# amazon-science/glass-text-spotting

Hardware: AMD Instinct MI355X
Metric: images/sec/GPU end-to-end spotting, 1000x1000, ~32 RoIs; 1/2/4/8 GPU scaling (higher is better)
Workload: dtype f32

## Files before the change

glass-text-spotting_amd/csrc/conv.hip:

```cpp
#include "splitk_common.h"
#include "common.h"
#include <cstdlib>

typedef float f32x16 __attribute__((ext_vector_type(16)));

struct ConvParams {
  const float* x;
  const float* w;
  const float* bias;
  const float* res;
  float* y;
  int N, H, W, Cin, Cout, KH, KW, sh, sw, ph, pw, Ho, Wo;
  int ldx, ldy, ycoff, ycs, relu, res_mode, ldr;
  int M, Ktot, nk, tiles_m, tiles_n, vec_epi;
  unsigned x_bytes, w_bytes;
  unsigned y_bytes, r_bytes;
  unsigned magic_cin, magic_kw;
  int ksplit;
  long split_y;
  int half_mode;
  int xh, yh, rh;
};

__device__ __forceinline__ float4 sel4(bool ok, float4 v) {
  return make_float4(ok ? v.x : 0.f, ok ? v.y : 0.f, ok ? v.z : 0.f, ok ? v.w : 0.f);
}


typedef unsigned u32x4 __attribute__((ext_vector_type(4)));
typedef unsigned u32x2 __attribute__((ext_vector_type(2)));

typedef _Float16 h8 __attribute__((ext_vector_type(8)));
typedef _Float16 h4 __attribute__((ext_vector_type(4)));

template <int WAVES_M, int WAVES_N, int TM, int TN, int NSTAGE, int MINW, int BK, int MODE, bool HALF>
__global__ __launch_bounds__(256, MINW) void conv_igemm_f32(ConvParams pin) {
  ConvParams p = pin;
  int kt0 = 0, kt1 = pin.nk;
  if (pin.ksplit > 1) {
    const int per = pin.nk / pin.ksplit;
    kt0 = (int)blockIdx.y * per;
    kt1 = kt0 + per;
    p.y += (long)blockIdx.y * pin.split_y;
  }
  constexpr bool FAST = MODE == 1, BUF = MODE != 0;
  constexpr int LDS_LD = HALF ? BK + 8 : BK + 4;
  constexpr int KCH = BK / 4;
  constexpr int RPP = 256 / KCH;
  constexpr int BM = WAVES_M * TM * 32;
  constexpr int BN = WAVES_N * TN * 32;
  constexpr int A_LOADS = BM / RPP;
  constexpr int B_LOADS = BN / RPP;
  constexpr int STAGE = (BM + BN) * LDS_LD;
  constexpr int ESZ = HALF ? 2 : 4;
  constexpr int CW = (NSTAGE * STAGE * ESZ >= BM * 68 * 4 && BN >= 64) ? 64 : 32;
  constexpr int SMEM_BYTES = NSTAGE * STAGE * ESZ > BM * (CW + 4) * 4 ? NSTAGE * STAGE * ESZ : BM * (CW + 4) * 4;
  __shared__ __attribute__((aligned(16))) unsigned char smem_raw[SMEM_BYTES];
  float* smem = reinterpret_cast<float*>(smem_raw);
  _Float16* hmem = reinterpret_cast<_Float16*>(smem_raw);

  const int nblk = gridDim.x, bid = blockIdx.x;
  const int xcd = bid & 7, q = nblk >> 3, r = nblk & 7;
  const int logical = (xcd < r ? xcd * (q + 1) : r * (q + 1) + (xcd - r) * q) + (bid >> 3);
  const int tile_m = logical / p.tiles_n;
  const int tile_n = logical - tile_m * p.tiles_n;
  const int m0 = tile_m * BM, n0 = tile_n * BN;

  const int tid = threadIdx.x, lane = tid & 63, wave = tid >> 6;
  const int wm = wave / WAVES_N, wn = wave % WAVES_N;
  const int cc = tid % KCH;
  const int r0 = tid / KCH;

  long a_base[A_LOADS];
  int a_hi0[A_LOADS], a_wi0[A_LOADS];
// ... 117 lines not shown
      float4 v = *reinterpret_cast<const float4*>(src);
      areg[i] = sel4(ok, v);
    }
#pragma unroll
    for (int i = 0; i < B_LOADS; ++i) {
      const bool ok = kvalid && b_ok[i];
      const float* src = ok ? (p.w + b_off[i] + (long)kt * BK) : p.w;
      float4 v = *reinterpret_cast<const float4*>(src);
      breg[i] = sel4(ok, v);
    }
  };
  auto load_tile = [&](int kt) {
    if constexpr (MODE == 1) load_tile_fast(kt); else if constexpr (MODE == 2) load_tile_buf(kt); else load_tile_generic(kt);
  };
  auto store_tile = [&](int stage) {
    if constexpr (HALF) {
      _Float16* As = hmem + stage * STAGE;
      _Float16* Bs = As + BM * LDS_LD;
      auto to_h4 = [](float4 v) { return h4{(_Float16)v.x, (_Float16)v.y, (_Float16)v.z, (_Float16)v.w}; };
#pragma unroll
      for (int i = 0; i < A_LOADS; ++i)
        *reinterpret_cast<h4*>(&As[(r0 + RPP * i) * LDS_LD + cc * 4]) = to_h4(areg[i]);
#pragma unroll
      for (int i = 0; i < B_LOADS; ++i)
        *reinterpret_cast<h4*>(&Bs[(r0 + RPP * i) * LDS_LD + cc * 4]) = to_h4(breg[i]);
    } else {
      float* As = smem + stage * STAGE;
      float* Bs = As + BM * LDS_LD;
#pragma unroll
      for (int i = 0; i < A_LOADS; ++i)
        *reinterpret_cast<float4*>(&As[(r0 + RPP * i) * LDS_LD + cc * 4]) = areg[i];
// ... 5 lines not shown

  f32x16 acc[TM][TN];
#pragma unroll
  for (int i = 0; i < TM; ++i)
#pragma unroll
    for (int j = 0; j < TN; ++j)
#pragma unroll
      for (int e = 0; e < 16; ++e) acc[i][j][e] = 0.f;

  const int frag_row = lane & 31;
  const int frag_k = (lane >> 5) * 4;
  const float* a_frag0 = smem + (wm * TM * 32 + frag_row) * LDS_LD + frag_k;
  const float* b_frag0 = smem + BM * LDS_LD + (wn * TN * 32 + frag_row) * LDS_LD + frag_k;
  const _Float16* a_frag0h = hmem + (wm * TM * 32 + frag_row) * LDS_LD + (lane >> 5) * 8;
  const _Float16* b_frag0h = hmem + BM * LDS_LD + (wn * TN * 32 + frag_row) * LDS_LD + (lane >> 5) * 8;

  load_tile(kt0);
  store_tile(0);
  __syncthreads();
  for (int kt = kt0; kt < kt1; ++kt) {
    const bool more = kt + 1 < kt1;
    if (BUF || more) load_tile(kt + 1);
    const int cur = NSTAGE == 2 ? ((kt - kt0) & 1) : 0;
    if constexpr (HALF) {
      const _Float16* a_frag = a_frag0h + cur * STAGE;
      const _Float16* b_frag = b_frag0h + cur * STAGE;
#pragma unroll
      for (int g = 0; g < BK / 16; ++g) {
        h8 af[TM], bf[TN];
#pragma unroll
        for (int i = 0; i < TM; ++i) af[i] = *reinterpret_cast<const h8*>(a_frag + i * 32 * LDS_LD + g * 16);
#pragma unroll
        for (int j = 0; j < TN; ++j) bf[j] = *reinterpret_cast<const h8*>(b_frag + j * 32 * LDS_LD + g * 16);
#pragma unroll
        for (int i = 0; i < TM; ++i)
#pragma unroll
          for (int j = 0; j < TN; ++j) acc[i][j] = __builtin_amdgcn_mfma_f32_32x32x16_f16(af[i], bf[j], acc[i][j], 0, 0, 0);
      }
    } else {
// ... 9 lines not shown
#pragma unroll
      for (int s = 0; s < 4; ++s) {
#pragma unroll
        for (int i = 0; i < TM; ++i) {
          const float a = s == 0 ? af[i].x : s == 1 ? af[i].y : s == 2 ? af[i].z : af[i].w;
#pragma unroll
          for (int j = 0; j < TN; ++j) {
            const float b = s == 0 ? bf[j].x : s == 1 ? bf[j].y : s == 2 ? bf[j].z : bf[j].w;
            acc[i][j] = __builtin_amdgcn_mfma_f32_32x32x2f32(a, b, acc[i][j], 0, 0, 0);
          }
        }
      }
    }
    }
    if constexpr (BUF) {
      constexpr int NL = A_LOADS + B_LOADS, NM = HALF ? (BK / 16) * TM * TN : (BK / 8) * 4 * TM * TN, PER = NM / NL > 0 ? NM / NL : 1;
#pragma unroll
      for (int i = 0; i < NL; ++i) {
        __builtin_amdgcn_sched_group_barrier(0x020, 1, 0);
        __builtin_amdgcn_sched_group_barrier(0x008, PER, 0);
      }
    }
    if (NSTAGE == 2) {
      if (more) store_tile((kt + 1 - kt0) & 1);
      __syncthreads();
    } else {
      __syncthreads();
      if (more) {
        store_tile(0);
        __syncthreads();
      }
// ... 124 lines not shown
  }
}

template <int WAVES_M, int WAVES_N, int TM, int TN, int NSTAGE, int MINW, int BK, bool HALF>
static int launch_conv_cfg(ConvParams& p, hipStream_t stream) {
  constexpr int BM = WAVES_M * TM * 32, BN = WAVES_N * TN * 32;
  p.tiles_m = cdiv(p.M, BM);
  p.tiles_n = cdiv(p.Cout, BN);
  const long nblk = (long)p.tiles_m * p.tiles_n;
  if (nblk <= 0 || nblk > 0x7fffffffL) {
    glass_set_error("glass_conv2d_nhwc: bad grid %ld", nblk);
    return GLASS_EINVAL;
  }
  p.nk = cdiv(p.Ktot, BK);
  const dim3 grid((unsigned)nblk, (unsigned)(p.ksplit > 1 ? p.ksplit : 1));
  if (p.x_bytes != 0 && p.Cin % BK == 0)
    hipLaunchKernelGGL((conv_igemm_f32<WAVES_M, WAVES_N, TM, TN, NSTAGE, MINW, BK, 1, HALF>), grid, dim3(256), 0, stream, p);
  else if (p.x_bytes != 0)
    hipLaunchKernelGGL((conv_igemm_f32<WAVES_M, WAVES_N, TM, TN, NSTAGE, MINW, BK, 2, HALF>), grid, dim3(256), 0, stream, p);
  else if constexpr (!HALF)
    hipLaunchKernelGGL((conv_igemm_f32<WAVES_M, WAVES_N, TM, TN, NSTAGE, MINW, BK, 0, false>), grid, dim3(256), 0, stream, p);
  else {
    glass_set_error("glass_conv2d_nhwc_f16: tensors of 2 GiB and more are not supported in the fp16 mode");
    return GLASS_EINVAL;
  }
  GLASS_CHECK_LAUNCH("glass_conv2d_nhwc");
  return GLASS_OK;
}

template <int WAVES_M, int WAVES_N, int TM, int TN, int NSTAGE, int MINW, int BK>
static int launch_conv_impl(ConvParams& p, hipStream_t stream) {
  return p.half_mode ? launch_conv_cfg<WAVES_M, WAVES_N, TM, TN, NSTAGE, MINW, BK, true>(p, stream)
                     : launch_conv_cfg<WAVES_M, WAVES_N, TM, TN, NSTAGE, MINW, BK, false>(p, stream);
}

static int conv_dispatch(const glass_conv_desc* d, const float* x, const float* w, const float* bias, const float* residual,
                         float* y, glass_stream_t stream, int half_mode, int h16_flags = 0);

extern "C" int glass_conv2d_nhwc(const glass_conv_desc* d, const float* x, const float* w, const float* bias,
                                 const float* residual, float* y, glass_stream_t stream) {
  return conv_dispatch(d, x, w, bias, residual, y, stream, 0);
}

extern "C" int glass_conv2d_nhwc_f16(const glass_conv_desc* d, const float* x, const float* w, const float* bias,
                                     const float* residual, float* y, glass_stream_t stream) {
  return conv_dispatch(d, x, w, bias, residual, y, stream, 1);
}

extern "C" int glass_conv2d_nhwc_h16(const glass_conv_desc* d, const void* x, const float* w, const float* bias,
                                     const void* residual, void* y, int flags, glass_stream_t stream) {
  GLASS_CHECK_ARG((flags & ~7) == 0, "glass_conv2d_nhwc_h16: unknown flags 0x%x", flags);
  return conv_dispatch(d, static_cast<const float*>(x), w, bias, static_cast<const float*>(residual), static_cast<float*>(y),
                       stream, 1, flags);
}

static int conv_dispatch(const glass_conv_desc* d, const float* x, const float* w, const float* bias, const float* residual,
                         float* y, glass_stream_t stream, int half_mode, int h16_flags) {
  GLASS_CHECK_ARG(d && x && w && y, "glass_conv2d_nhwc: null pointer");
  GLASS_CHECK_ARG(d->Cin > 0 && d->Cin % 4 == 0, "glass_conv2d_nhwc: Cin=%d must be a positive multiple of 4", d->Cin);
  GLASS_CHECK_ARG(d->ldx % 4 == 0 && d->ldx >= d->Cin, "glass_conv2d_nhwc: ldx=%d", d->ldx);
  GLASS_CHECK_ARG(d->N >= 0 && d->H > 0 && d->W > 0 && d->Cout > 0 && d->KH > 0 && d->KW > 0, "glass_conv2d_nhwc: bad dims");
  GLASS_CHECK_ARG(d->stride_h > 0 && d->stride_w > 0, "glass_conv2d_nhwc: bad stride");
  GLASS_CHECK_ARG(d->Ho == (d->H + 2 * d->pad_h - d->KH) / d->stride_h + 1 &&
                      d->Wo == (d->W + 2 * d->pad_w - d->KW) / d->stride_w + 1,
                  "glass_conv2d_nhwc: Ho/Wo (%d,%d) inconsistent with input/kernel/stride/pad", d->Ho, d->Wo);
  GLASS_CHECK_ARG(d->y_cstride >= 1 && d->ldy >= 1 && d->y_coff >= 0, "glass_conv2d_nhwc: bad output strides");
  GLASS_CHECK_ARG((long)d->y_coff + (long)(d->Cout - 1) * d->y_cstride < (long)d->ldy,
                  "glass_conv2d_nhwc: output channel window (y_coff=%d, Cout=%d, y_cstride=%d) exceeds ldy=%d", d->y_coff,
                  d->Cout, d->y_cstride, d->ldy);
  GLASS_CHECK_ARG(d->res_mode == 0 || d->ldr >= d->Cout, "glass_conv2d_nhwc: residual ldr=%d < Cout=%d", d->ldr, d->Cout);
  GLASS_CHECK_ARG(d->res_mode == 0 || residual != nullptr, "glass_conv2d_nhwc: res_mode set but residual is null");
  GLASS_CHECK_ARG(d->res_mode != 2 || (d->Ho % 2 == 0 && d->Wo % 2 == 0), "glass_conv2d_nhwc: upsampled residual needs even Ho/Wo");
  GLASS_CHECK_ARG(((uintptr_t)x & 15) == 0 && ((uintptr_t)w & 15) == 0, "glass_conv2d_nhwc: x/w must be 16-byte aligned");
  if (d->N == 0) return GLASS_OK;
  ConvParams p;
  p.half_mode = half_mode;
  p.xh = h16_flags & 1; p.yh = (h16_flags >> 1) & 1; p.rh = (h16_flags >> 2) & 1;
  const long xes = p.xh ? 2 : 4, yes = p.yh ? 2 : 4, res_ = p.rh ? 2 : 4;
  p.x = x; p.w = w; p.bias = bias; p.res = residual; p.y = y;
  p.N = d->N; p.H = d->H; p.W = d->W; p.Cin = d->Cin; p.Cout = d->Cout; p.KH = d->KH; p.KW = d->KW;
  p.sh = d->stride_h; p.sw = d->stride_w; p.ph = d->pad_h; p.pw = d->pad_w; p.Ho = d->Ho; p.Wo = d->Wo;
  p.ldx = d->ldx; p.ldy = d->ldy; p.ycoff = d->y_coff; p.ycs = d->y_cstride; p.relu = d->relu;
  p.res_mode = d->res_mode; p.ldr = d->ldr;
  const long M = (long)d->N * d->Ho * d->Wo;
  GLASS_CHECK_ARG(M < 0x7fffffffL, "glass_conv2d_nhwc: too many output pixels");
  p.M = (int)M;
  p.Ktot = d->KH * d->KW * d->Cin;
  p.ksplit = 1; p.split_y = 0;
  {
    const long xb = (long)d->N * d->H * d->W * d->ldx * 4, wb = (long)d->Cout * p.Ktot * 4;
    const bool small = xb < 0x7fffff00L && wb < 0x7fffff00L;
// ... 55 lines not shown
                                        glass_stream_t stream) {
  GLASS_CHECK_ARG(d && x && w && y && workspace, "glass_conv2d_nhwc_splitk: null pointer");
  GLASS_CHECK_ARG(glass_conv2d_splitk_supported(d, splits),
                  "glass_conv2d_nhwc_splitk: needs Cin %% 32 == 0, (KH KW Cin / 32) %% splits == 0, 2 <= splits <= 32, res_mode 0/1 and "
                  "operands < 2 GiB (got Cin=%d k=%dx%d splits=%d res_mode=%d)", d->Cin, d->KH, d->KW, splits, d->res_mode);
  GLASS_CHECK_ARG(d->Ho == (d->H + 2 * d->pad_h - d->KH) / d->stride_h + 1 && d->Wo == (d->W + 2 * d->pad_w - d->KW) / d->stride_w + 1,
                  "glass_conv2d_nhwc_splitk: Ho/Wo (%d,%d) inconsistent with input/kernel/stride/pad", d->Ho, d->Wo);
  GLASS_CHECK_ARG(d->y_cstride >= 1 && d->y_coff >= 0 && (long)d->y_coff + (long)(d->Cout - 1) * d->y_cstride < (long)d->ldy,
                  "glass_conv2d_nhwc_splitk: output channel window exceeds ldy=%d", d->ldy);
  GLASS_CHECK_ARG(d->res_mode == 0 || (residual != nullptr && d->ldr >= d->Cout), "glass_conv2d_nhwc_splitk: bad residual");
  GLASS_CHECK_ARG(workspace_bytes >= glass_conv2d_splitk_workspace_bytes(d, splits), "glass_conv2d_nhwc_splitk: workspace too small");
  GLASS_CHECK_ARG((((uintptr_t)x | (uintptr_t)w | (uintptr_t)workspace) & 15) == 0, "glass_conv2d_nhwc_splitk: x / w / workspace must be 16-byte aligned");
  GLASS_CHECK_ARG(d->relu >= 0 && d->relu <= 2, "glass_conv2d_nhwc_splitk: relu must be 0, 1 or 2");
  const long M = (long)d->N * d->Ho * d->Wo;
  ConvParams p;
  p.half_mode = 0; p.xh = p.yh = p.rh = 0;
  p.x = x; p.w = w; p.bias = nullptr; p.res = nullptr; p.y = static_cast<float*>(workspace);
  p.N = d->N; p.H = d->H; p.W = d->W; p.Cin = d->Cin; p.Cout = d->Cout; p.KH = d->KH; p.KW = d->KW;
  p.sh = d->stride_h; p.sw = d->stride_w; p.ph = d->pad_h; p.pw = d->pad_w; p.Ho = d->Ho; p.Wo = d->Wo;
  p.ldx = d->ldx; p.ldy = d->Cout; p.ycoff = 0; p.ycs = 1; p.relu = 0; p.res_mode = 0; p.ldr = 0;
  p.M = (int)M; p.Ktot = d->KH * d->KW * d->Cin; p.ksplit = splits; p.split_y = M * d->Cout;
  p.x_bytes = (unsigned)((long)d->N * d->H * d->W * d->ldx * 4);
  p.w_bytes = (unsigned)((long)d->Cout * p.Ktot * 4);
  p.magic_cin = (unsigned)(0x100000000ULL / (unsigned long long)d->Cin);
  p.magic_kw = (unsigned)(0x100000000ULL / (unsigned long long)d->KW);
  p.vec_epi = d->Cout % 4 == 0 ? 1 : 0;
  p.y_bytes = (unsigned)(M * d->Cout * 4);
  p.r_bytes = 0;
  hipStream_t s = (hipStream_t)stream;
  const int rc = d->Cout <= 32 ? launch_conv_impl<4, 1, 1, 1, 1, 4, 32>(p, s)
                               : launch_conv_impl<2, 2, 1, 1, 1, 8, 32>(p, s);
// ... 7 lines not shown
```

glass-text-spotting_amd/csrc/pointwise_split.hip:

```cpp
#include "wino_common.h"

typedef float f32x4 __attribute__((ext_vector_type(4)));
typedef __bf16 bf16x8 __attribute__((ext_vector_type(8)));
typedef unsigned u32x2 __attribute__((ext_vector_type(2)));

namespace {

constexpr int SN = 128;
constexpr int SK = 32;

struct PwsParams {
  const float* x; const void* u; const float* bias; const float* res; float* y;
  int M, H, W, Ho, Wo, Cin, Cout, stride, nk;
  int ldx, ldy, ycoff, ldr, relu, res_mode;
  int tiles_m, tiles_n;
  unsigned x_bytes, u_bytes, y_bytes, r_bytes;
  unsigned magic_hw, magic_w;
  unsigned long long* dbg;
  const float* x2; int nk1, ldx2; unsigned x2_bytes;
};

#ifdef GLASS_PWS_STAMPS
unsigned long long* g_pws_dbg = nullptr;
#define PWS_STAMP(k) { __builtin_amdgcn_sched_barrier(0); const unsigned long long tn = __builtin_amdgcn_s_memtime(); st[k] += tn - tlast; tlast = tn; __builtin_amdgcn_sched_barrier(0); }
#else
#define PWS_STAMP(k) {}
#endif

typedef float f32x2 __attribute__((ext_vector_type(2)));
typedef __bf16 bf16x2 __attribute__((ext_vector_type(2)));
__device__ __forceinline__ void split3_pair(float v0, float v1, unsigned& hp, unsigned& mp, unsigned& lp) {
  hp = __builtin_bit_cast(unsigned, __builtin_convertvector((f32x2{v0, v1}), bf16x2));
  const float r0 = v0 - __builtin_bit_cast(float, hp << 16), r1 = v1 - __builtin_bit_cast(float, hp & 0xffff0000u);
  mp = __builtin_bit_cast(unsigned, __builtin_convertvector((f32x2{r0, r1}), bf16x2));
  const float l0 = r0 - __builtin_bit_cast(float, mp << 16), l1 = r1 - __builtin_bit_cast(float, mp & 0xffff0000u);
  lp = __builtin_bit_cast(unsigned, __builtin_convertvector((f32x2{l0, l1}), bf16x2));
}

template <int PB, int NPROD, bool DUAL = false>
__global__ __launch_bounds__(256, 2) void conv1x1_pw_split(PwsParams p) {
  constexpr int PX = 16 * PB;
  constexpr int XL = PX / 32;
  constexpr int NW = 4;
  constexpr int PLANE = PX * 64;
  constexpr int STAGE = 3 * PLANE;
  __shared__ __attribute__((aligned(16))) unsigned char smem[2 * STAGE];

  const int nblk = gridDim.x, bid = blockIdx.x;
  const int xcd = bid & 7, q8 = nblk >> 3, r8 = nblk & 7;
  const int logical = (xcd < r8 ? xcd * (q8 + 1) : r8 * (q8 + 1) + (xcd - r8) * q8) + (bid >> 3);
  const int tile_m = logical / p.tiles_n;
  const int tile_n = logical - tile_m * p.tiles_n;
// ... 330 lines not shown
```

glass-text-spotting_amd/glass_amd/_lib.py:

```python
from __future__ import annotations

import ctypes
import glob
import os
import subprocess
from typing import List, Optional

_PKG = os.path.dirname(os.path.abspath(__file__))
_ROOT = os.path.dirname(_PKG)
CSRC = os.path.join(_ROOT, "csrc")
INCLUDE = os.path.join(os.path.dirname(_ROOT), "include")
SO_PATH = os.environ.get("GLASS_HIP_LIB") or os.path.join(_ROOT, "libglass_hip.so")

EXPORTS = [
    "glass_last_error", "glass_abi_version", "glass_device_count", "glass_conv2d_nhwc", "glass_conv2d_nhwc_f16", "glass_conv2d_nhwc_h16", "glass_local_stem_supported", "glass_local_stem_fused", "glass_local_stem_fused_h16", "glass_backbone_stem_supported", "glass_backbone_stem_fused", "glass_conv3x3_winograd43_body_nhwc", "glass_winograd43_splitk_supported", "glass_winograd43_splitk_workspace_bytes", "glass_conv3x3_winograd43_splitk_nhwc", "glass_roi_align_rotated_up2", "glass_conv2d_splitk_supported", "glass_conv2d_splitk_workspace_bytes", "glass_conv2d_nhwc_splitk", "glass_conv3x3_winograd_body_nhwc",
    "glass_pointwise_supported", "glass_pointwise_weight_floats", "glass_pointwise_pack_weights", "glass_conv1x1_pointwise_nhwc",
    "glass_pointwise_split_supported", "glass_pointwise_split_weight_bytes", "glass_pointwise_split_pack_weights", "glass_conv1x1_pointwise_split_nhwc", "glass_pointwise_split_dual_supported", "glass_conv1x1_pointwise_split_dual_nhwc",
    "glass_conv_h16_supported", "glass_conv_h16_weight_halves", "glass_conv_h16_pack_weights", "glass_conv2d_nhwc_h16_packed",
    "glass_winograd_supported", "glass_winograd_block_channels", "glass_winograd_weight_floats", "glass_winograd_pack_weights", "glass_conv3x3_winograd_nhwc",
    "glass_winograd43_supported", "glass_winograd43_weight_floats", "glass_winograd43_pack_weights", "glass_conv3x3_winograd43_nhwc",
    "glass_maxpool2d_nhwc", "glass_maxpool2d_nhwc_h16", "glass_roi_align_rotated_h16", "glass_pixel_shuffle2x_nhwc", "glass_sigmoid_inplace", "glass_paste_rotated_masks", "glass_mul_inplace", "glass_cast_f32_to_f16",
    "glass_preprocess_image", "glass_image_u8hwc_to_chw_resized", "glass_roi_align_rotated",
    "glass_rpn_workspace_bytes", "glass_rpn_topk_decode", "glass_rotated_nms_select", "glass_pairwise_iou_rotated", "glass_detections_finalize", "glass_postprocess_words", "glass_postprocess_words_dense_workspace_bytes", "glass_postprocess_words_dense", "glass_text_argmax", "glass_pack_word_records",
    "glass_box_decode", "glass_gc_attention_inplace", "glass_mean_over_h", "glass_bilstm_workspace_bytes", "glass_bilstm_recurrence",
    "glass_bilstm_persistent_workspace_bytes", "glass_bilstm_recurrence_persistent", "glass_recurrence_status", "glass_recurrence_test_hook",
    "glass_decode_persistent_supported", "glass_decode_persistent_workspace_bytes", "glass_attention_decode_persistent",
    "glass_decode_workspace_bytes", "glass_attention_decode", "glass_decode_step_workspace_bytes", "glass_attention_decode_step",
    "glass_lexicon_match_workspace_bytes", "glass_lexicon_match",
    "glass_lexicon_match_weighted_workspace_bytes", "glass_lexicon_match_weighted",
    "glass_rrc_pair_areas_workspace_bytes", "glass_rrc_pair_areas", "glass_rrc_match_workspace_bytes", "glass_rrc_match",
# ... 110 lines not shown
```

glass-text-spotting_amd/glass_amd/ops/native.py:

```python
from __future__ import annotations

import collections
import ctypes
import math
import os
import struct
import threading
from typing import List, NamedTuple, Optional, Sequence, Tuple

import numpy as np
import torch

from .._lib import GlassLibraryError, check, lib

c_int, c_float, c_void_p = ctypes.c_int, ctypes.c_float, ctypes.c_void_p


class ConvDesc(ctypes.Structure):
    _fields_ = [(n, c_int) for n in (
        "N", "H", "W", "Cin", "Cout", "KH", "KW", "stride_h", "stride_w", "pad_h", "pad_w", "Ho", "Wo",
        "ldx", "ldy", "y_coff", "y_cstride", "relu", "res_mode", "ldr")]


class RoiAlignDesc(ctypes.Structure):
# ... 65 lines not shown
        raise GlassLibraryError(f"unknown recurrent routing {v!r} (steps | persistent | 2x1 | 2x2 | 1x1)")
    return (nd, ng)


def _parse_split(v) -> int:
    try:
        n = int(v)
    except (TypeError, ValueError):
        n = -1
    if n not in (0, 6, 9):
        raise GlassLibraryError(f"unknown 1x1 split routing {v!r} (0 | 9 | 6)")
    return n


class Routing:
    __slots__ = ("precision", "winograd", "f43", "pw", "h16", "local_stem", "stem", "ragged", "pooled_fusion", "rnn", "splitk", "small_grid", "split")

    def __init__(self, precision: Optional[str] = None, winograd: Optional[bool] = None, f43: Optional[bool] = None, pw=None,
                 h16: Optional[bool] = None, local_stem: Optional[bool] = None, stem: Optional[bool] = None,
                 ragged: Optional[bool] = None, pooled_fusion: Optional[bool] = None, rnn=None,
                 splitk: Optional[bool] = None, small_grid: Optional[bool] = None, split: Optional[int] = None):
        e = os.environ.get
        self.precision = precision or e("GLASS_CONV_PRECISION", "fp32")
        if self.precision not in _PRECISIONS:
            raise GlassLibraryError(f"unknown conv precision {self.precision!r}")
        self.winograd = (e("GLASS_WINOGRAD", "1") != "0") if winograd is None else bool(winograd)
        self.f43 = (e("GLASS_WINOGRAD43", "1") != "0") if f43 is None else bool(f43)
        self.pw = {"0": False, "all": "all"}.get(e("GLASS_POINTWISE", "1"), True) if pw is None else (pw if pw == "all" else bool(pw))
        self.h16 = (e("GLASS_CONV_H16", "1") != "0") if h16 is None else bool(h16)
        self.local_stem = (e("GLASS_LOCAL_STEM", "1") != "0") if local_stem is None else bool(local_stem)
        self.stem = (e("GLASS_BACKBONE_STEM", "1") != "0") if stem is None else bool(stem)
        self.ragged = (e("GLASS_W43_RAGGED", "1") != "0") if ragged is None else bool(ragged)
        self.pooled_fusion = (e("GLASS_POOLED_FUSION", "1") != "0") if pooled_fusion is None else bool(pooled_fusion)
        self.rnn = _parse_rnn(e("GLASS_RNN", "1x1")) if rnn is None else _parse_rnn(rnn)
        self.splitk = (e("GLASS_SPLITK", "1") != "0") if splitk is None else bool(splitk)
        self.small_grid = (e("GLASS_SMALL_GRID", "1") != "0") if small_grid is None else bool(small_grid)
        self.split = _parse_split(e("GLASS_PW_SPLIT", "9") if split is None else split)

    def replace(self, **kw) -> "Routing":
        r = Routing.__new__(Routing)
        for k in Routing.__slots__:
            setattr(r, k, kw.pop(k, getattr(self, k)))
        if kw:
            raise TypeError(f"unknown routing fields {sorted(kw)}")
        if r.precision not in _PRECISIONS:
            raise GlassLibraryError(f"unknown conv precision {r.precision!r}")
        r.split = _parse_split(r.split)
        r.rnn = _parse_rnn(r.rnn)
        return r

    @property
    def act_dtype(self) -> torch.dtype:
# ... 102 lines not shown

def _use_f43(N: int, H: int, W: int, Cout: int, Cin: int, body: bool = False) -> bool:
    t4 = ((H + 3) // 4) * (W // 4 if body else (W + 3) // 4)
    waste = (t4 * 16.0) / (((H + 1) // 2) * ((W + 1) // 2) * 4.0)
    return waste <= 1.25 and _wino_workgroups(4, N, H, W, Cout, Cout % 128 == 0 and Cin % 32 == 0, body) >= 192


NUM_CUS = 256


def _use_split(px: int, Cin: int, Cout: int) -> bool:
    blocks = -(-px // 64) * (Cout // 128)
    if 192 <= blocks < 384 and Cin >= 512:
        return True
    return blocks >= 384 and (Cin >= 128 or px >= 262144)


def _small_grid_3x3(N: int, H: int, W: int, Cout: int, Cin: int, can_body: bool, f43_ok: bool):
    def rounds(blocks):
        return -(-blocks // NUM_CUS)
    cands = []
    wide = Cout % 128 == 0 and Cin % 32 == 0
    for body in ((False, True) if can_body else (False,)):
        strip = 20.0 if body else 0.0
        if f43_ok and (not body or W % 4 == 1):
            blocks = _wino_workgroups(4, N, H, W, Cout, wide, body)
            cands.append((rounds(blocks) * ((10 + 0.34 * Cin) if wide else (9 + 0.56 * Cin)) + strip, "f43", body))
        blocks = _wino_workgroups(2, N, H, W, Cout, wide, body)
        cands.append((rounds(blocks) * ((9 + 0.30 * Cin) if wide else 3.0 * Cin) + strip, "f22", body))
    t, kind, body = min(cands)
# ... 191 lines not shown
        if ragged:
            return ConvPlan("winograd43r", "glass_conv3x3_winograd43_body_nhwc", True, strip=True)
        return ConvPlan("winograd43", "glass_conv3x3_winograd43_nhwc", True)
    if forced == "f43":
        raise GlassLibraryError("winograd='f43' but glass_winograd43_supported() rejects this layer")
    if use_wino and three and L.glass_winograd_supported(dp):
        path = "winograd128" if L.glass_winograd_block_channels(Cout, Cin) == 128 else "winograd"
        if f22_body:
            return ConvPlan(path + "r", "glass_conv3x3_winograd_body_nhwc", False, strip=True)
        return ConvPlan(path, "glass_conv3x3_winograd_nhwc", False)
    if forced:
        raise GlassLibraryError("winograd=True but glass_winograd_supported() rejects this layer")
    splits = _splitk_slices(rt, px, KH * KW * Cin, Cin, Cout) if (res_mode in (0, 1) or res_dtype is None) else 0
    if splits > 1 and out_dtype == torch.float32 and L.glass_conv2d_splitk_supported(dp, splits):
        return ConvPlan("direct", "glass_conv2d_nhwc_splitk", splits=splits)
    return ConvPlan("direct", "glass_conv2d_nhwc")


def conv2d_nhwc(x: torch.Tensor, w, bias: Optional[torch.Tensor] = None, *, stride=1, padding=0,
                relu: int = 0, residual: Optional[torch.Tensor] = None, res_mode: int = 0,
                out: Optional[torch.Tensor] = None, out_coff: int = 0, out_cstride: int = 1,
                cin: Optional[int] = None, winograd: Optional[bool] = None, out_dtype: Optional[torch.dtype] = None,
                precision: Optional[str] = None, routing: Optional[Routing] = None, f43k=None) -> torch.Tensor:
    wt = w.raw if isinstance(w, ConvWeight) else _f32c(w, "w")
    rt = routing if routing is not None else routing_of(w)
    if precision is not None and precision != rt.precision:
        rt = rt.replace(precision=precision)
    _fhc(x, "x")
    N, H, W, ldx = x.shape
    Cout, KH, KW, Cin = wt.shape
# ... 27 lines not shown
    xt = x
    if cast:
        xt = torch.empty(x.shape, dtype=torch.float16, device=x.device)
        check(L.glass_cast_f32_to_f16(c_void_p(_dev(x, "x")), c_void_p(_dev(xt)), ctypes.c_int64(x.numel()),
                                      c_void_p(stream_handle())), "glass_cast_f32_to_f16")
    args = [ctypes.byref(d), c_void_p(_dev(xt, "x")), c_void_p(_dev(wt if pack is None else _packed(w, wt, pack), "w")),
            c_void_p(_dev(bias, "bias") if bias is not None else None),
            c_void_p(_dev(residual, "residual") if residual is not None else None), c_void_p(_dev(out, "out"))]
    tail = [] if flags is None else [flags]
    if splits:
        nbytes = int(getattr(L, _WORKSPACE_BYTES[entry])(ctypes.byref(d), splits))
        ws = torch.empty((nbytes,), dtype=torch.uint8, device=x.device)
        tail = [splits] + tail + [c_void_p(_dev(ws)), ctypes.c_int64(nbytes)]
    check(getattr(L, entry)(*args, *tail, c_void_p(stream_handle())), entry)
    if strip:
        _last_column_strip(x, _packed(w, wt, "col1"), bias, residual, out, d, out_coff)
    return out


def prepare_dual_weights(w1, w2) -> Optional["ConvWeight"]:
    r1, r2 = _raw(w1), _raw(w2)
    load = getattr(_TLS, "load", None)
    rt = load if load is not None else _DEFAULT
    if (rt.precision != "fp32" or rt.split != 9 or not r1.is_cuda or r1.shape[1:3] != (1, 1) or r2.shape[1:3] != (1, 1) or
            r1.shape[0] != r2.shape[0] or r1.shape[0] % 128 or r1.shape[3] % 32 or r2.shape[3] % 32):
        return None
    cw = ConvWeight(torch.cat([r1, r2], dim=3).contiguous(), routing=load)
    cw.packs["pws"] = winograd_pack(cw.raw, "pws")
    if load is None:
        torch.cuda.current_stream().synchronize()
    return cw
# ... 22 lines not shown
    Cout, Cin2 = w.raw.shape[0], x2.shape[3]
    Cin1 = w.raw.shape[3] - Cin2
    Ho, Wo = conv_out_size(H, W, 1, 1, stride, 0)
    if tuple(x2.shape[:3]) != (N, Ho, Wo) or ldx != Cin1:
        raise GlassLibraryError(f"conv1x1_dual_nhwc: x1 {tuple(x1.shape)} (stride {stride}) and x2 {tuple(x2.shape)} do not share an output grid / weight {tuple(w.raw.shape)}")
    out = torch.empty((N, Ho, Wo, Cout), dtype=torch.float32, device=x1.device)
    d = ConvDesc(N, H, W, Cin1, Cout, 1, 1, stride, stride, 0, 0, Ho, Wo, ldx, Cout, 0, 1, relu, 0, 0)
    _TLS.last_path = "pointwise_split"
    check(lib().glass_conv1x1_pointwise_split_dual_nhwc(
        ctypes.byref(d), c_void_p(_dev(x1, "x1")), c_void_p(_dev(x2, "x2")), int(Cin2), int(x2.shape[3]), c_void_p(_dev(_packed(w, w.raw, "pws"), "w")),
        c_void_p(_dev(bias, "bias") if bias is not None else None), c_void_p(_dev(out, "out")), c_void_p(stream_handle())),
        "glass_conv1x1_pointwise_split_dual_nhwc")
    return out


def _last_column_strip(x: torch.Tensor, wcol: torch.Tensor, bias, residual, out: torch.Tensor, d: ConvDesc, out_coff: int) -> None:
    N, H, W, Cin, Cout = d.N, d.H, d.W, d.Cin, d.Cout
    assert d.ldx == Cin, "the caller routes only dense inputs here"
    ds = ConvDesc(N, H, 1, 2 * Cin, Cout, 3, 1, 1, 1, 1, 0, H, 1, W * d.ldx, W * d.ldy, (W - 1) * d.ldy + out_coff, 1, d.relu,
                  d.res_mode, W * d.ldr if d.res_mode else 0)
    isz = x.element_size()
    xp = _dev(x, "x") + (W - 2) * d.ldx * isz
    rp = (_dev(residual, "residual") + (W - 1) * d.ldr * residual.element_size()) if (residual is not None and d.res_mode) else None
    check(lib().glass_conv2d_nhwc(ctypes.byref(ds), c_void_p(xp), c_void_p(_dev(wcol, "w")),
                                  c_void_p(_dev(bias, "bias") if bias is not None else None), c_void_p(rp), c_void_p(_dev(out, "out")),
                                  c_void_p(stream_handle())), "glass_conv2d_nhwc(last column)")


def _splitk_slices(rt: Routing, M: int, Ktot: int, Cin: int, Cout: int, want_time: bool = False):
    if not rt.splitk or rt.precision != "fp32" or Cin % 32 != 0 or M <= 0:
        return (0, float("inf")) if want_time else 0
    nk = Ktot // 32
    if nk < 16:
        return (0, float("inf")) if want_time else 0
    tiles = -(-M // 128) if Cout <= 32 else -(-M // 64) * -(-Cout // 64)

    def t(s):
        wpc = max(1.0, tiles * s / NUM_CUS)
        extra = 0.0 if s == 1 else 2.0 * s * M * Cout * 4 / 4e6 + 5.0 + 0.3 * s
        return nk / s * (0.75 if wpc <= 1.0 else 0.3 + 0.45 * wpc) + extra
    t1 = t(1)
# ... 810 lines not shown
```

include/glass_hip.h:

```cpp
#ifndef GLASS_HIP_H
#define GLASS_HIP_H

#include <stddef.h>
#include <stdint.h>

#ifdef __cplusplus
extern "C" {
#endif

#define GLASS_OK 0
#define GLASS_EINVAL (-1)
#define GLASS_EHIP (-2)
#define GLASS_ENOMEM (-3)

typedef void* glass_stream_t;

const char* glass_last_error(void);
int glass_abi_version(void);
int glass_device_count(void);

typedef struct glass_conv_desc {
  int N, H, W, Cin;
  int Cout, KH, KW;
  int stride_h, stride_w, pad_h, pad_w;
  int Ho, Wo;
  int ldx;
  int ldy, y_coff, y_cstride;
  int relu;
  int res_mode;
  int ldr;
} glass_conv_desc;

int glass_conv2d_nhwc(const glass_conv_desc* d, const float* x, const float* w, const float* bias,
                      const float* residual, float* y, glass_stream_t stream);

int glass_conv2d_nhwc_f16(const glass_conv_desc* d, const float* x, const float* w, const float* bias,
                          const float* residual, float* y, glass_stream_t stream);

int glass_conv2d_nhwc_h16(const glass_conv_desc* d, const void* x, const float* w, const float* bias, const void* residual,
                          void* y, int flags, glass_stream_t stream);

int glass_conv_h16_supported(const glass_conv_desc* d, int flags);
size_t glass_conv_h16_weight_halves(int Cout, int KH, int KW, int Cin);
int glass_conv_h16_pack_weights(const float* w, int Cout, int KH, int KW, int Cin, void* u_packed, glass_stream_t stream);
int glass_conv2d_nhwc_h16_packed(const glass_conv_desc* d, const void* x, const void* u_packed, const float* bias,
                                 const void* residual, void* y, int flags, glass_stream_t stream);

int glass_winograd_supported(const glass_conv_desc* d);
int glass_winograd_block_channels(int Cout, int Cin);
size_t glass_winograd_weight_floats(int Cout, int Cin);
int glass_winograd_pack_weights(const float* w, int Cout, int Cin, float* u_packed, glass_stream_t stream);
int glass_conv3x3_winograd_nhwc(const glass_conv_desc* d, const float* x, const float* u_packed, const float* bias,
// ... 221 lines not shown
```

Baseline: 315.2.

## Add bf16x3 split-precision MFMA path to the fp32 implicit-GEMM conv kernel

Adds a SPLIT mode to the implicit-GEMM conv kernel. Each fp32 operand tile is split into three bf16 planes (high, mid, low) in LDS, and the product is accumulated with nine bf16 32x32x16 MFMAs per k-group instead of the slow fp32 32x32x2 MFMA. This is meant to get near-fp32 accuracy at higher matrix throughput. In exchange LDS use triples, occupancy may drop, and the split adds conversion ALU work. The Python router enables it by default for non-3x3 fp32 convs above size thresholds, including the last-column strip path.

Result: no change. 316.4 (median of 6 runs) (+0.4%).

```diff
diff --git a/glass-text-spotting_amd/csrc/bf16_split.h b/glass-text-spotting_amd/csrc/bf16_split.h
--- /dev/null
+++ b/glass-text-spotting_amd/csrc/bf16_split.h
@@ -0,0 +1,20 @@
+#pragma once
+
+typedef __bf16 bf16x8 __attribute__((ext_vector_type(8)));
+
+namespace {
+
+typedef float split_f32x2 __attribute__((ext_vector_type(2)));
+typedef __bf16 split_bf16x2 __attribute__((ext_vector_type(2)));
+__device__ __forceinline__ unsigned cvt_pk_bf16(float v0, float v1) {
+  return __builtin_bit_cast(unsigned, __builtin_convertvector((split_f32x2{v0, v1}), split_bf16x2));
+}
+__device__ __forceinline__ void split3_pair(float v0, float v1, unsigned& hp, unsigned& mp, unsigned& lp) {
+  hp = cvt_pk_bf16(v0, v1);
+  const float r0 = v0 - __builtin_bit_cast(float, hp << 16), r1 = v1 - __builtin_bit_cast(float, hp & 0xffff0000u);
+  mp = cvt_pk_bf16(r0, r1);
+  const float l0 = r0 - __builtin_bit_cast(float, mp << 16), l1 = r1 - __builtin_bit_cast(float, mp & 0xffff0000u);
+  lp = cvt_pk_bf16(l0, l1);
+}
+
+}
diff --git a/glass-text-spotting_amd/csrc/conv.hip b/glass-text-spotting_amd/csrc/conv.hip
--- a/glass-text-spotting_amd/csrc/conv.hip
+++ b/glass-text-spotting_amd/csrc/conv.hip
@@ -1,5 +1,6 @@
 #include "splitk_common.h"
 #include "common.h"
+#include "bf16_split.h"
 #include <cstdlib>
 
 typedef float f32x16 __attribute__((ext_vector_type(16)));
@@ -20,6 +21,7 @@
   long split_y;
   int half_mode;
   int xh, yh, rh;
+  int split_mode;
 };
 
 __device__ __forceinline__ float4 sel4(bool ok, float4 v) {
@@ -33,8 +35,14 @@
 typedef _Float16 h8 __attribute__((ext_vector_type(8)));
 typedef _Float16 h4 __attribute__((ext_vector_type(4)));
 
-template <int WAVES_M, int WAVES_N, int TM, int TN, int NSTAGE, int MINW, int BK, int MODE, bool HALF>
+constexpr int conv_split_minw(int BM, int BN, int NSTAGE, int BK, int MINW) {
+  const int bytes = NSTAGE * 3 * (BM + BN) * (BK + 8) * 2;
+  return bytes > 65536 ? 0 : (163840 / bytes < MINW ? 163840 / bytes : MINW);
+}
+
+template <int WAVES_M, int WAVES_N, int TM, int TN, int NSTAGE, int MINW, int BK, int MODE, bool HALF, bool SPLIT = false>
 __global__ __launch_bounds__(256, MINW) void conv_igemm_f32(ConvParams pin) {
+  static_assert(!SPLIT || (MODE == 1 && !HALF), "the bf16-split mode exists for the uniform-tap load path only");
   ConvParams p = pin;
   int kt0 = 0, kt1 = pin.nk;
   if (pin.ksplit > 1) {
@@ -44,20 +52,22 @@
     p.y += (long)blockIdx.y * pin.split_y;
   }
   constexpr bool FAST = MODE == 1, BUF = MODE != 0;
-  constexpr int LDS_LD = HALF ? BK + 8 : BK + 4;
+  constexpr int LDS_LD = (HALF || SPLIT) ? BK + 8 : BK + 4;
   constexpr int KCH = BK / 4;
   constexpr int RPP = 256 / KCH;
   constexpr int BM = WAVES_M * TM * 32;
   constexpr int BN = WAVES_N * TN * 32;
   constexpr int A_LOADS = BM / RPP;
   constexpr int B_LOADS = BN / RPP;
-  constexpr int STAGE = (BM + BN) * LDS_LD;
-  constexpr int ESZ = HALF ? 2 : 4;
-  constexpr int CW = (NSTAGE * STAGE * ESZ >= BM * 68 * 4 && BN >= 64) ? 64 : 32;
+  constexpr int PLANE = (BM + BN) * LDS_LD;
+  constexpr int STAGE = (SPLIT ? 3 : 1) * PLANE;
+  constexpr int ESZ = (HALF || SPLIT) ? 2 : 4;
+  constexpr int CW = (NSTAGE * STAGE * ESZ >= BM * 68 * 4 && BN % 64 == 0) ? 64 : 32;
   constexpr int SMEM_BYTES = NSTAGE * STAGE * ESZ > BM * (CW + 4) * 4 ? NSTAGE * STAGE * ESZ : BM * (CW + 4) * 4;
   __shared__ __attribute__((aligned(16))) unsigned char smem_raw[SMEM_BYTES];
   float* smem = reinterpret_cast<float*>(smem_raw);
   _Float16* hmem = reinterpret_cast<_Float16*>(smem_raw);
+  __bf16* bmem = reinterpret_cast<__bf16*>(smem_raw);
 
   const int nblk = gridDim.x, bid = blockIdx.x;
   const int xcd = bid & 7, q = nblk >> 3, r = nblk & 7;
@@ -205,7 +215,22 @@
     if constexpr (MODE == 1) load_tile_fast(kt); else if constexpr (MODE == 2) load_tile_buf(kt); else load_tile_generic(kt);
   };
   auto store_tile = [&](int stage) {
-    if constexpr (HALF) {
+    if constexpr (SPLIT) {
+      __bf16* As = bmem + stage * STAGE;
+      __bf16* Bs = As + BM * LDS_LD;
+      auto put = [](__bf16* dst, float4 v) {
+        unsigned h0, m0, l0, h1, m1, l1;
+        split3_pair(v.x, v.y, h0, m0, l0);
+        split3_pair(v.z, v.w, h1, m1, l1);
+        *reinterpret_cast<u32x2*>(dst) = u32x2{h0, h1};
+        *reinterpret_cast<u32x2*>(dst + PLANE) = u32x2{m0, m1};
+        *reinterpret_cast<u32x2*>(dst + 2 * PLANE) = u32x2{l0, l1};
+      };
+#pragma unroll
+      for (int i = 0; i < A_LOADS; ++i) put(&As[(r0 + RPP * i) * LDS_LD + cc * 4], areg[i]);
+#pragma unroll
+      for (int i = 0; i < B_LOADS; ++i) put(&Bs[(r0 + RPP * i) * LDS_LD + cc * 4], breg[i]);
+    } else if constexpr (HALF) {
       _Float16* As = hmem + stage * STAGE;
       _Float16* Bs = As + BM * LDS_LD;
       auto to_h4 = [](float4 v) { return h4{(_Float16)v.x, (_Float16)v.y, (_Float16)v.z, (_Float16)v.w}; };
@@ -241,6 +266,8 @@
   const float* b_frag0 = smem + BM * LDS_LD + (wn * TN * 32 + frag_row) * LDS_LD + frag_k;
   const _Float16* a_frag0h = hmem + (wm * TM * 32 + frag_row) * LDS_LD + (lane >> 5) * 8;
   const _Float16* b_frag0h = hmem + BM * LDS_LD + (wn * TN * 32 + frag_row) * LDS_LD + (lane >> 5) * 8;
+  const __bf16* a_frag0s = bmem + (wm * TM * 32 + frag_row) * LDS_LD + (lane >> 5) * 8;
+  const __bf16* b_frag0s = bmem + BM * LDS_LD + (wn * TN * 32 + frag_row) * LDS_LD + (lane >> 5) * 8;
 
   load_tile(kt0);
   store_tile(0);
@@ -249,7 +276,30 @@
     const bool more = kt + 1 < kt1;
     if (BUF || more) load_tile(kt + 1);
     const int cur = NSTAGE == 2 ? ((kt - kt0) & 1) : 0;
-    if constexpr (HALF) {
+    if constexpr (SPLIT) {
+      const __bf16* a_frag = a_frag0s + cur * STAGE;
+      const __bf16* b_frag = b_frag0s + cur * STAGE;
+#pragma unroll
+      for (int g = 0; g < BK / 16; ++g) {
+        bf16x8 af[TM][3], bf[TN][3];
+#pragma unroll
+        for (int q = 0; q < 3; ++q) {
+#pragma unroll
+          for (int i = 0; i < TM; ++i) af[i][q] = *reinterpret_cast<const bf16x8*>(a_frag + q * PLANE + i * 32 * LDS_LD + g * 16);
+#pragma unroll
+          for (int j = 0; j < TN; ++j) bf[j][q] = *reinterpret_cast<const bf16x8*>(b_frag + q * PLANE + j * 32 * LDS_LD + g * 16);
+        }
+#pragma unroll
+        for (int t = 0; t < 9; ++t) {
+          const int qa = 2 - t / 3, qb = 2 - t % 3;
+#pragma unroll
+          for (int i = 0; i < TM; ++i)
+#pragma unroll
+            for (int j = 0; j < TN; ++j)
+              acc[i][j] = __builtin_amdgcn_mfma_f32_32x32x16_bf16(af[i][qa], bf[j][qb], acc[i][j], 0, 0, 0);
+        }
+      }
+    } else if constexpr (HALF) {
       const _Float16* a_frag = a_frag0h + cur * STAGE;
       const _Float16* b_frag = b_frag0h + cur * STAGE;
 #pragma unroll
@@ -289,7 +339,7 @@
     }
     }
     if constexpr (BUF) {
-      constexpr int NL = A_LOADS + B_LOADS, NM = HALF ? (BK / 16) * TM * TN : (BK / 8) * 4 * TM * TN, PER = NM / NL > 0 ? NM / NL : 1;
+      constexpr int NL = A_LOADS + B_LOADS, NM = SPLIT ? (BK / 16) * 9 * TM * TN : HALF ? (BK / 16) * TM * TN : (BK / 8) * 4 * TM * TN, PER = NM / NL > 0 ? NM / NL : 1;
 #pragma unroll
       for (int i = 0; i < NL; ++i) {
         __builtin_amdgcn_sched_group_barrier(0x020, 1, 0);
@@ -444,7 +494,19 @@
   }
   p.nk = cdiv(p.Ktot, BK);
   const dim3 grid((unsigned)nblk, (unsigned)(p.ksplit > 1 ? p.ksplit : 1));
-  if (p.x_bytes != 0 && p.Cin % BK == 0)
+  if (p.split_mode) {
+    constexpr int MINW_S = conv_split_minw(BM, BN, NSTAGE, BK, MINW);
+    if constexpr (!HALF && MINW_S > 0) {
+      if (p.x_bytes == 0 || p.Cin % BK != 0) {
+        glass_set_error("glass_conv2d_nhwc_bs: needs Cin %% %d == 0 and operands < 2 GiB (glass_conv2d_bs_supported)", BK);
+        return GLASS_EINVAL;
+      }
+      hipLaunchKernelGGL((conv_igemm_f32<WAVES_M, WAVES_N, TM, TN, NSTAGE, MINW_S, BK, 1, false, true>), grid, dim3(256), 0, stream, p);
+    } else {
+      glass_set_error("glass_conv2d_nhwc_bs: this tile configuration has no bf16-split form");
+      return GLASS_EINVAL;
+    }
+  } else if (p.x_bytes != 0 && p.Cin % BK == 0)
     hipLaunchKernelGGL((conv_igemm_f32<WAVES_M, WAVES_N, TM, TN, NSTAGE, MINW, BK, 1, HALF>), grid, dim3(256), 0, stream, p);
   else if (p.x_bytes != 0)
     hipLaunchKernelGGL((conv_igemm_f32<WAVES_M, WAVES_N, TM, TN, NSTAGE, MINW, BK, 2, HALF>), grid, dim3(256), 0, stream, p);
@@ -465,7 +527,7 @@
 }
 
 static int conv_dispatch(const glass_conv_desc* d, const float* x, const float* w, const float* bias, const float* residual,
-                         float* y, glass_stream_t stream, int half_mode, int h16_flags = 0);
+                         float* y, glass_stream_t stream, int half_mode, int h16_flags = 0, int split_mode = 0);
 
 extern "C" int glass_conv2d_nhwc(const glass_conv_desc* d, const float* x, const float* w, const float* bias,
                                  const float* residual, float* y, glass_stream_t stream) {
@@ -475,6 +537,21 @@
 extern "C" int glass_conv2d_nhwc_f16(const glass_conv_desc* d, const float* x, const float* w, const float* bias,
                                      const float* residual, float* y, glass_stream_t stream) {
   return conv_dispatch(d, x, w, bias, residual, y, stream, 1);
+}
+
+extern "C" int glass_conv2d_bs_supported(const glass_conv_desc* d) {
+  if (!d) return 0;
+  const long K = (long)d->KH * d->KW * d->Cin;
+  return d->N > 0 && d->H > 0 && d->W > 0 && d->Cout > 0 && d->KH > 0 && d->KW > 0 && d->Cin > 0 && d->Cin % 32 == 0 &&
+         d->ldx % 4 == 0 && d->ldx >= d->Cin && (long)d->N * d->H * d->W * d->ldx * 4 < 0x7fffff00L &&
+         (long)d->Cout * K * 4 < 0x7fffff00L;
+}
+
+extern "C" int glass_conv2d_nhwc_bs(const glass_conv_desc* d, const float* x, const float* w, const float* bias,
+                                    const float* residual, float* y, glass_stream_t stream) {
+  GLASS_CHECK_ARG(d == nullptr || d->N == 0 || glass_conv2d_bs_supported(d),
+                  "glass_conv2d_nhwc_bs: needs Cin %% 32 == 0 and operands < 2 GiB (glass_conv2d_bs_supported)");
+  return conv_dispatch(d, x, w, bias, residual, y, stream, 0, 0, 1);
 }
 
 extern "C" int glass_conv2d_nhwc_h16(const glass_conv_desc* d, const void* x, const float* w, const float* bias,
@@ -485,7 +562,7 @@
 }
 
 static int conv_dispatch(const glass_conv_desc* d, const float* x, const float* w, const float* bias, const float* residual,
-                         float* y, glass_stream_t stream, int half_mode, int h16_flags) {
+                         float* y, glass_stream_t stream, int half_mode, int h16_flags, int split_mode) {
   GLASS_CHECK_ARG(d && x && w && y, "glass_conv2d_nhwc: null pointer");
   GLASS_CHECK_ARG(d->Cin > 0 && d->Cin % 4 == 0, "glass_conv2d_nhwc: Cin=%d must be a positive multiple of 4", d->Cin);
   GLASS_CHECK_ARG(d->ldx % 4 == 0 && d->ldx >= d->Cin, "glass_conv2d_nhwc: ldx=%d", d->ldx);
@@ -505,6 +582,7 @@
   if (d->N == 0) return GLASS_OK;
   ConvParams p;
   p.half_mode = half_mode;
+  p.split_mode = split_mode;
   p.xh = h16_flags & 1; p.yh = (h16_flags >> 1) & 1; p.rh = (h16_flags >> 2) & 1;
   const long xes = p.xh ? 2 : 4, yes = p.yh ? 2 : 4, res_ = p.rh ? 2 : 4;
   p.x = x; p.w = w; p.bias = bias; p.res = residual; p.y = y;
@@ -590,7 +668,7 @@
   GLASS_CHECK_ARG(d->relu >= 0 && d->relu <= 2, "glass_conv2d_nhwc_splitk: relu must be 0, 1 or 2");
   const long M = (long)d->N * d->Ho * d->Wo;
   ConvParams p;
-  p.half_mode = 0; p.xh = p.yh = p.rh = 0;
+  p.half_mode = 0; p.split_mode = 0; p.xh = p.yh = p.rh = 0;
   p.x = x; p.w = w; p.bias = nullptr; p.res = nullptr; p.y = static_cast<float*>(workspace);
   p.N = d->N; p.H = d->H; p.W = d->W; p.Cin = d->Cin; p.Cout = d->Cout; p.KH = d->KH; p.KW = d->KW;
   p.sh = d->stride_h; p.sw = d->stride_w; p.ph = d->pad_h; p.pw = d->pad_w; p.Ho = d->Ho; p.Wo = d->Wo;
diff --git a/glass-text-spotting_amd/csrc/pointwise_split.hip b/glass-text-spotting_amd/csrc/pointwise_split.hip
--- a/glass-text-spotting_amd/csrc/pointwise_split.hip
+++ b/glass-text-spotting_amd/csrc/pointwise_split.hip
@@ -1,7 +1,7 @@
 #include "wino_common.h"
+#include "bf16_split.h"
 
 typedef float f32x4 __attribute__((ext_vector_type(4)));
-typedef __bf16 bf16x8 __attribute__((ext_vector_type(8)));
 typedef unsigned u32x2 __attribute__((ext_vector_type(2)));
 
 namespace {
@@ -27,15 +27,6 @@
 #define PWS_STAMP(k) {}
 #endif
 
-typedef float f32x2 __attribute__((ext_vector_type(2)));
-typedef __bf16 bf16x2 __attribute__((ext_vector_type(2)));
-__device__ __forceinline__ void split3_pair(float v0, float v1, unsigned& hp, unsigned& mp, unsigned& lp) {
-  hp = __builtin_bit_cast(unsigned, __builtin_convertvector((f32x2{v0, v1}), bf16x2));
-  const float r0 = v0 - __builtin_bit_cast(float, hp << 16), r1 = v1 - __builtin_bit_cast(float, hp & 0xffff0000u);
-  mp = __builtin_bit_cast(unsigned, __builtin_convertvector((f32x2{r0, r1}), bf16x2));
-  const float l0 = r0 - __builtin_bit_cast(float, mp << 16), l1 = r1 - __builtin_bit_cast(float, mp & 0xffff0000u);
-  lp = __builtin_bit_cast(unsigned, __builtin_convertvector((f32x2{l0, l1}), bf16x2));
-}
 
 template <int PB, int NPROD, bool DUAL = false>
 __global__ __launch_bounds__(256, 2) void conv1x1_pw_split(PwsParams p) {
diff --git a/glass-text-spotting_amd/glass_amd/_lib.py b/glass-text-spotting_amd/glass_amd/_lib.py
--- a/glass-text-spotting_amd/glass_amd/_lib.py
+++ b/glass-text-spotting_amd/glass_amd/_lib.py
@@ -13,7 +13,7 @@
 SO_PATH = os.environ.get("GLASS_HIP_LIB") or os.path.join(_ROOT, "libglass_hip.so")
 
 EXPORTS = [
-    "glass_last_error", "glass_abi_version", "glass_device_count", "glass_conv2d_nhwc", "glass_conv2d_nhwc_f16", "glass_conv2d_nhwc_h16", "glass_local_stem_supported", "glass_local_stem_fused", "glass_local_stem_fused_h16", "glass_backbone_stem_supported", "glass_backbone_stem_fused", "glass_conv3x3_winograd43_body_nhwc", "glass_winograd43_splitk_supported", "glass_winograd43_splitk_workspace_bytes", "glass_conv3x3_winograd43_splitk_nhwc", "glass_roi_align_rotated_up2", "glass_conv2d_splitk_supported", "glass_conv2d_splitk_workspace_bytes", "glass_conv2d_nhwc_splitk", "glass_conv3x3_winograd_body_nhwc",
+    "glass_last_error", "glass_abi_version", "glass_device_count", "glass_conv2d_nhwc", "glass_conv2d_nhwc_f16", "glass_conv2d_bs_supported", "glass_conv2d_nhwc_bs", "glass_conv2d_nhwc_h16", "glass_local_stem_supported", "glass_local_stem_fused", "glass_local_stem_fused_h16", "glass_backbone_stem_supported", "glass_backbone_stem_fused", "glass_conv3x3_winograd43_body_nhwc", "glass_winograd43_splitk_supported", "glass_winograd43_splitk_workspace_bytes", "glass_conv3x3_winograd43_splitk_nhwc", "glass_roi_align_rotated_up2", "glass_conv2d_splitk_supported", "glass_conv2d_splitk_workspace_bytes", "glass_conv2d_nhwc_splitk", "glass_conv3x3_winograd_body_nhwc",
     "glass_pointwise_supported", "glass_pointwise_weight_floats", "glass_pointwise_pack_weights", "glass_conv1x1_pointwise_nhwc",
     "glass_pointwise_split_supported", "glass_pointwise_split_weight_bytes", "glass_pointwise_split_pack_weights", "glass_conv1x1_pointwise_split_nhwc", "glass_pointwise_split_dual_supported", "glass_conv1x1_pointwise_split_dual_nhwc",
     "glass_conv_h16_supported", "glass_conv_h16_weight_halves", "glass_conv_h16_pack_weights", "glass_conv2d_nhwc_h16_packed",
diff --git a/glass-text-spotting_amd/glass_amd/ops/native.py b/glass-text-spotting_amd/glass_amd/ops/native.py
--- a/glass-text-spotting_amd/glass_amd/ops/native.py
+++ b/glass-text-spotting_amd/glass_amd/ops/native.py
@@ -103,12 +103,13 @@
 
 
 class Routing:
-    __slots__ = ("precision", "winograd", "f43", "pw", "h16", "local_stem", "stem", "ragged", "pooled_fusion", "rnn", "splitk", "small_grid", "split")
+    __slots__ = ("precision", "winograd", "f43", "pw", "h16", "local_stem", "stem", "ragged", "pooled_fusion", "rnn", "splitk", "small_grid", "split", "igemm_split")
 
     def __init__(self, precision: Optional[str] = None, winograd: Optional[bool] = None, f43: Optional[bool] = None, pw=None,
                  h16: Optional[bool] = None, local_stem: Optional[bool] = None, stem: Optional[bool] = None,
                  ragged: Optional[bool] = None, pooled_fusion: Optional[bool] = None, rnn=None,
-                 splitk: Optional[bool] = None, small_grid: Optional[bool] = None, split: Optional[int] = None):
+                 splitk: Optional[bool] = None, small_grid: Optional[bool] = None, split: Optional[int] = None,
+                 igemm_split: Optional[bool] = None):
         e = os.environ.get
         self.precision = precision or e("GLASS_CONV_PRECISION", "fp32")
         if self.precision not in _PRECISIONS:
@@ -125,6 +126,8 @@
         self.splitk = (e("GLASS_SPLITK", "1") != "0") if splitk is None else bool(splitk)
         self.small_grid = (e("GLASS_SMALL_GRID", "1") != "0") if small_grid is None else bool(small_grid)
         self.split = _parse_split(e("GLASS_PW_SPLIT", "9") if split is None else split)
+        self.igemm_split = ({"0": False, "all": "all"}.get(e("GLASS_IGEMM_SPLIT", "1"), True) if igemm_split is None
+                            else (igemm_split if igemm_split == "all" else bool(igemm_split)))
 
     def replace(self, **kw) -> "Routing":
         r = Routing.__new__(Routing)
@@ -257,6 +260,14 @@
     if 192 <= blocks < 384 and Cin >= 512:
         return True
     return blocks >= 384 and (Cin >= 128 or px >= 262144)
+
+
+def _use_igemm_split(rt: "Routing", px: int, KH: int, KW: int, Cin: int, Cout: int) -> bool:
+    if rt.precision != "fp32" or rt.split != 9 or not rt.igemm_split:
+        return False
+    if rt.igemm_split == "all":
+        return True
+    return KH * KW * Cin >= 256 and px >= 16384 and not (64 < Cout <= 96) and not (KH == 3 and KW == 3)
 
 
 def _small_grid_3x3(N: int, H: int, W: int, Cout: int, Cin: int, can_body: bool, f43_ok: bool):
@@ -478,6 +489,9 @@
     splits = _splitk_slices(rt, px, KH * KW * Cin, Cin, Cout) if (res_mode in (0, 1) or res_dtype is None) else 0
     if splits > 1 and out_dtype == torch.float32 and L.glass_conv2d_splitk_supported(dp, splits):
         return ConvPlan("direct", "glass_conv2d_nhwc_splitk", splits=splits)
+    if (not forced and out_dtype == torch.float32 and _use_igemm_split(rt, px, KH, KW, Cin, Cout) and
+            L.glass_conv2d_bs_supported(dp)):
+        return ConvPlan("direct", "glass_conv2d_nhwc_bs")
     return ConvPlan("direct", "glass_conv2d_nhwc")
 
 
@@ -535,7 +549,7 @@
         tail = [splits] + tail + [c_void_p(_dev(ws)), ctypes.c_int64(nbytes)]
     check(getattr(L, entry)(*args, *tail, c_void_p(stream_handle())), entry)
     if strip:
-        _last_column_strip(x, _packed(w, wt, "col1"), bias, residual, out, d, out_coff)
+        _last_column_strip(x, _packed(w, wt, "col1"), bias, residual, out, d, out_coff, rt)
     return out
 
 
@@ -588,7 +602,8 @@
     return out
 
 
-def _last_column_strip(x: torch.Tensor, wcol: torch.Tensor, bias, residual, out: torch.Tensor, d: ConvDesc, out_coff: int) -> None:
+def _last_column_strip(x: torch.Tensor, wcol: torch.Tensor, bias, residual, out: torch.Tensor, d: ConvDesc, out_coff: int,
+                       rt: Optional[Routing] = None) -> None:
     N, H, W, Cin, Cout = d.N, d.H, d.W, d.Cin, d.Cout
     assert d.ldx == Cin, "the caller routes only dense inputs here"
     ds = ConvDesc(N, H, 1, 2 * Cin, Cout, 3, 1, 1, 1, 1, 0, H, 1, W * d.ldx, W * d.ldy, (W - 1) * d.ldy + out_coff, 1, d.relu,
@@ -596,9 +611,14 @@
     isz = x.element_size()
     xp = _dev(x, "x") + (W - 2) * d.ldx * isz
     rp = (_dev(residual, "residual") + (W - 1) * d.ldr * residual.element_size()) if (residual is not None and d.res_mode) else None
-    check(lib().glass_conv2d_nhwc(ctypes.byref(ds), c_void_p(xp), c_void_p(_dev(wcol, "w")),
-                                  c_void_p(_dev(bias, "bias") if bias is not None else None), c_void_p(rp), c_void_p(_dev(out, "out")),
-                                  c_void_p(stream_handle())), "glass_conv2d_nhwc(last column)")
+    L = lib()
+    bs = (rt is not None and _use_igemm_split(rt, N * H, 3, 1, 2 * Cin, Cout) and x.dtype == torch.float32 and
+          out.dtype == torch.float32 and (residual is None or residual.dtype == torch.float32) and
+          L.glass_conv2d_bs_supported(ctypes.byref(ds)))
+    entry = L.glass_conv2d_nhwc_bs if bs else L.glass_conv2d_nhwc
+    check(entry(ctypes.byref(ds), c_void_p(xp), c_void_p(_dev(wcol, "w")),
+                c_void_p(_dev(bias, "bias") if bias is not None else None), c_void_p(rp), c_void_p(_dev(out, "out")),
+                c_void_p(stream_handle())), "glass_conv2d_nhwc(last column)")
 
 
 def _splitk_slices(rt: Routing, M: int, Ktot: int, Cin: int, Cout: int, want_time: bool = False):
diff --git a/include/glass_hip.h b/include/glass_hip.h
--- a/include/glass_hip.h
+++ b/include/glass_hip.h
@@ -36,6 +36,10 @@
 
 int glass_conv2d_nhwc_f16(const glass_conv_desc* d, const float* x, const float* w, const float* bias,
                           const float* residual, float* y, glass_stream_t stream);
+
+int glass_conv2d_bs_supported(const glass_conv_desc* d);
+int glass_conv2d_nhwc_bs(const glass_conv_desc* d, const float* x, const float* w, const float* bias,
+                         const float* residual, float* y, glass_stream_t stream);
 
 int glass_conv2d_nhwc_h16(const glass_conv_desc* d, const void* x, const float* w, const float* bias, const void* residual,
                           void* y, int flags, glass_stream_t stream);
```
